# MJavaadAkhtar/GCN-max-cut

Hardware: AMD Instinct MI355X
Metric: training epochs/sec (n=1000 d=7 graphs) (higher is better)
Workload: dtype f32; 1 GPU; 160 x n=1000 d=7 regular graphs per GPU (BASELINE configs[3] on one GPU; 160 graphs per step), GCN 1000->500->3, batched steps, Adam lr 1e-3; graphs_per_gpu=160, rows_per_gpu=160000, nnz_per_gpu=1120000, hidden_dim=500, mode=batched, epoch_graphs=160, parallelism=single

## Files before the change

gcn-max-cut_amd/csrc/api.hip:

```cpp
#include "launchers.h"
#include <stdlib.h>

namespace {

int g_fuse = -1;
bool fuse_enabled() {
    if (g_fuse < 0) {
        g_fuse = 1;
#ifdef GMC_TUNING
        const char *e = getenv("GMC_FUSE");
        if (e && e[0] == '0') g_fuse = 0;
#endif
    }
    return g_fuse != 0;
}

struct Plan {
    int fs;
    bool fused;
    bool head_in_bwd;
    int zparts;
    int slices;
    int chunks;
};

Plan plan(const gmc_batch *b, int F, float dropout_p, bool fuse, bool train_step, bool dense = false,
          bool hard_loss = true) {
    Plan p{};
    p.zparts = 1;
    if (dense) return p;
    const bool dropout = dropout_p > 0.f;
    const GmcLdsGeom g = gmc_lds_geometry(b, F);
    bool lds = g.fits && !(g.ovf && (!fuse || dropout));
#ifdef GMC_TUNING
    static const bool forced_rows = [] {
        const char *e = getenv("GMC_SPMM_ALGO");
        return e && e[0] == 'r';
    }();
    if (forced_rows) lds = false;
#endif
    if (!lds) return p;
    p.fs = g.fs;
    p.slices = g.slices;
    p.chunks = gmc_dw1_chunks(b->B, true, g.slices);
    p.fused = fuse && !dropout;
    if (!dropout) p.zparts = gmc_lds_groups(b, F);
    p.head_in_bwd = train_step && hard_loss && p.fused && p.chunks == 1 && gmc_bwd1_takes_head(b);
    return p;
}

struct Workspace {
    Plan plan;
    long ld;
    float *T0;
    float *H;
    float *Z0;
    float *GY2;
    float *part;
    float *db2part;
    float *dw1part;
    float *W2s;
    size_t bytes;
};

bool dropout_on(const gmc_model *m) { return m->dropout_p > 0.f; }
int loss_kind_of(const gmc_model *m) { return (m->flags & GMC_MODEL_LOSS_EXPECTED) ? GMC_LOSS_EXPECTED_CUT : GMC_LOSS_CUT; }
unsigned long long dropout_seed(const gmc_model *m) { return ((unsigned long long)m->dropout_seed_hi << 32) | m->dropout_seed_lo; }

size_t align_up(size_t x) { return (x + 255) & ~(size_t)255; }

Workspace carve(const gmc_batch *b, const gmc_model *m, int training, void *base, bool train_step = false,
                bool dense = false) {
    Workspace w{};
    size_t off = 0;
    auto take = [&](size_t floats) {
        float *p = base ? reinterpret_cast<float *>(static_cast<char *>(base) + off) : nullptr;
        off += align_up(floats * sizeof(float));
        return p;
    };
// ... 18 lines not shown
    return w;
}

int check(const gmc_batch *b, const gmc_model *m, bool dense = false) {
    if (!b || !m) return GMC_ERR_NULL;
    if (b->abi != GMC_VERSION || m->abi != GMC_VERSION) return GMC_ERR_ABI;
    if (!b->goff || !b->rowptr || !b->gcol || !b->lcol || !b->dinv) return GMC_ERR_NULL;
    if (!m->W1 || !m->b1 || !m->W2 || !m->b2) return GMC_ERR_NULL;
    if (m->K != 3) return GMC_ERR_CLASSES;
    if (b->B < 0 || b->R < 0 || b->nnz < 0 || m->N <= 0 || m->F <= 0) return GMC_ERR_SHAPE;
    if (m->F % 4 || m->F > GMC_MAX_HIDDEN) return GMC_ERR_UNSUPPORTED;
    if (!(m->dropout_p >= 0.f && m->dropout_p < 1.f)) return GMC_ERR_SHAPE;
    if (m->W1_slab && !gmc_aligned16(m->W1_slab)) return GMC_ERR_ALIGN;
    if (b->B > 0 && (b->n_max < 3 || b->n_max > GMC_MAX_GRAPH_NODES)) return GMC_ERR_GRAPH_SIZE;
    if (!dense && b->n_max > m->N) return GMC_ERR_SHAPE;
    return GMC_OK;
}

int group_rows(const gmc_batch *b) { return b->uniform_n > 0 ? b->uniform_n : b->n_max; }


int aggregate(const gmc_batch *b, const Workspace &w, const float *X, float *Y, int F, const float *bias, int relu,
              const float *W2, float *Z0, int tag, hipStream_t st) {
    if (w.plan.fs)
        return gmc_spmm_lds_launch(b, X, w.ld, 1, 0, 0, b->dinv, bias, relu, Y, w.ld, 1, F, W2, Z0, tag, st);
    return gmc_spmm_launch(b->rowptr, b->gcol, nullptr, b->dinv, X, w.ld, bias, relu, Y, w.ld, b->R, F,
                           group_rows(b), W2, Z0, tag, st);
}

int forward_body(const gmc_batch *b, const gmc_model *m, const Workspace &w, hipStream_t st, const float *X = nullptr,
                 long ldx = 0) {
    const int F = m->F;
    if (w.plan.fused)
        return gmc_fwd1_lds_launch(b, m->W1, m->b1, m->W2, w.H, w.Z0, F, st, m->W1_slab, m->N);
    const int fs = w.plan.fs;
    int rc = X ? gmc_gemm_launch(0, 0, b->R, F, m->N, X, ldx, m->W1, F, b->dinv, w.T0, w.ld, st)
             : fs ? gmc_spmm_lds_launch(b, m->W1, F, 0, 1, 1, b->dinv, nullptr, 0, w.T0, w.ld, 1, F, nullptr,
                                        nullptr, GMC_K_GATHER_W1, st)
                  : gmc_spmm_launch(b->rowptr, b->lcol, b->vals, b->dinv, m->W1, F, nullptr, 0, w.T0, w.ld,
                                    b->R, F, group_rows(b), nullptr, nullptr, GMC_K_GATHER_W1, st);
    if (rc) return rc;
    if (dropout_on(m)) {
        rc = aggregate(b, w, w.T0, w.H, F, m->b1, 1, nullptr, nullptr, GMC_K_AGG_FWD, st);
        if (rc) return rc;
        rc = gmc_dropout_launch(w.H, b->R, F, fs, w.ld, m->dropout_p, dropout_seed(m), st);
        if (rc) return rc;
        return gmc_hw2_rows_launch(w.H, b->dinv, m->W2, w.Z0, b->R, F, fs, w.ld, st);
    }
    return aggregate(b, w, w.T0, w.H, F, m->b1, 1, m->W2, w.Z0, GMC_K_AGG_FWD, st);
}

struct AdamFuse {
    float *param = nullptr, *m = nullptr, *v = nullptr;
    double lr = 0, beta1 = 0, beta2 = 0, eps = 0;
    int *step_counter = nullptr;
    float *w1_slab = nullptr;
};

int backward_body(const gmc_batch *b, const gmc_model *m, const Workspace &w, float *grad,
                  hipStream_t st, const AdamFuse *af = nullptr, const float *loss_tail = nullptr,
                  const gmc_bwd1_head *head = nullptr, const float *X = nullptr, long ldx = 0, float *dX = nullptr,
                  long lddx = 0) {
    const long F = m->F;
    float *dW1 = grad, *db1 = grad + (long)m->N * F, *dW2 = db1 + F, *db2 = dW2 + F * 3;
    float *Gs = w.T0, *U = w.H;
    const float *W2b = m->W2;
    if (dropout_on(m)) {
// ... 79 lines not shown
}

extern "C" int gmc_probe_end(int32_t *tags, float *ms, int32_t max) {
    g_probe.on = false;
    const int n = (int)g_probe.used;
    if (n > 0) {
        hipError_t e = hipEventSynchronize(g_probe.pool[n - 1].b);
        if (e != hipSuccess) return -(int)e - 1000;
    }
    for (int i = 0; i < n && i < max; ++i) {
        float t = 0.f;
        (void)hipEventElapsedTime(&t, g_probe.pool[i].a, g_probe.pool[i].b);
        if (tags) tags[i] = g_probe.pool[i].tag;
        if (ms) ms[i] = t;
    }
    return n;
}

extern "C" int gmc_probe_flavours(int32_t *words, int32_t max) {
    if (g_probe.on) return GMC_ERR_UNSUPPORTED;
    const int n = (int)g_probe.used;
    for (int i = 0; i < n && i < max; ++i)
        if (words) words[i] = g_probe.pool[i].flv;
    return n;
}

extern "C" int gmc_lds_flavours(const gmc_batch *batch, int32_t F, int32_t one_graph_step, int32_t *words, int32_t max) {
    if (!batch) return GMC_ERR_NULL;
    if (batch->abi != GMC_VERSION) return GMC_ERR_ABI;
    if (F <= 0 || F % 4 || F > GMC_MAX_HIDDEN || max < 0 || batch->B < 0) return GMC_ERR_SHAPE;
    int out[6], n = 0;
    const Plan fused = plan(batch, F, 0.f, true, one_graph_step != 0), unfused = plan(batch, F, 0.f, false, false);
    if (fused.fused) {
        out[n++] = gmc_fwd1_flavour(batch, F);
        out[n++] = gmc_bwd1_flavour(batch, F, fused.head_in_bwd);
    }
    if (unfused.fs) {
        out[n++] = gmc_spmm_lds_flavour(batch, F, 1, 1, false);
        out[n++] = gmc_spmm_lds_flavour(batch, F, 0, 0, true);
        out[n++] = gmc_spmm_lds_flavour(batch, F, 0, 0, false);
        out[n++] = gmc_dw1_lds_flavour(batch, F);
    }
    for (int i = 0; i < n && i < max; ++i)
        if (words) words[i] = out[i];
    return n;
}

extern "C" int gmc_set_fuse(int on) {
    const int prev = fuse_enabled() ? 1 : 0;
    g_fuse = on ? 1 : 0;
    return prev;
}

extern "C" int gmc_version(void) { return GMC_VERSION; }

extern "C" const char *gmc_error_string(int code) {
    switch (code) {
        case GMC_OK: return "ok";
        case GMC_ERR_NULL: return "required pointer is NULL";
        case GMC_ERR_SHAPE: return "negative or inconsistent sizes";
        case GMC_ERR_CLASSES: return "number_classes must be 3 (override_fixed_nodes is 3-wide)";
        case GMC_ERR_ALIGN: return "pointer or leading dimension not 16-byte aligned";
        case GMC_ERR_WORKSPACE: return "workspace too small";
        case GMC_ERR_GRAPH_SIZE: return "graph has fewer than 3 or more than GMC_MAX_GRAPH_NODES nodes";
        case GMC_ERR_UNSUPPORTED: return "unsupported shape (the hidden width F must be a multiple of 4 and <= 4096 = GMC_MAX_HIDDEN)";
        case GMC_ERR_LOSS: return "unknown loss kind (GMC_LOSS_CUT = 0, GMC_LOSS_EXPECTED_CUT = 1)";
        case GMC_ERR_ABI: return "gmc_batch.abi / gmc_model.abi differs from the library's GMC_VERSION: rebuild the caller against this include/gcnmaxcut.h";
// ... 172 lines not shown
```

gcn-max-cut_amd/csrc/fwd1_lds.hip:

```cpp
#include "lds_tile.h"

#ifdef GMC_STAMP
extern "C" int gmc_debug_read_stamps_fwd(unsigned long long *out, int n) {
    return (int)hipMemcpyFromSymbol(out, HIP_SYMBOL(g_stamps), sizeof(unsigned long long) * n);
}
#endif

namespace {

template <int FS, int W, int ACC, bool HAS_VAL, int NS, bool OVF>
__global__ GMC_LDS_BOUNDS void fwd1_lds_kernel(TileArgs a) {
    STAMP_DECL;
    MARK(0);
    extern __shared__ __attribute__((aligned(16))) float lds[];
    constexpr int Q = FS / 4;
    constexpr int kRowsPerPass = kThreads / Q;
    constexpr int NT = (ACC * kRowsPerPass * (W / 8) + kThreads - 1) / kThreads;
    const int total = a.b.B * a.groups;
    const int it0 = (int)blockIdx.x * a.items_per_wg, it1 = min(total, it0 + a.items_per_wg);
    if (it0 >= it1) return;
    const int per = (a.slices + a.groups - 1) / a.groups;

    const int TF = (int)tile_floats(a.b.n_max, FS);
    float *bufA = lds, *bufB = lds + TF;
    unsigned short *nb = reinterpret_cast<unsigned short *>(lds + 2 * TF);
    constexpr bool CSL = W == 16;
    float4 *cst = reinterpret_cast<float4 *>(nb + (size_t)a.b.n_max * W);
    const int q = threadIdx.x % Q, lrow = threadIdx.x / Q;
    constexpr bool ovf = OVF;
    auto col_consts = [&](int cc) {
        float4 c = gmc::f4_zero();
        if (cc < a.F) {
            if (a.W2) { c.x = a.W2[(long)cc * 3]; c.y = a.W2[(long)cc * 3 + 1]; c.z = a.W2[(long)cc * 3 + 2]; }
            if (a.bias) c.w = a.bias[cc];
        }
        return c;
    };

    constexpr int kSlicesPerWin = kThreads / FS;
    auto load_window = [&](int win) {
        const int cc = win * kThreads + (int)threadIdx.x;
// ... 61 lines not shown
            for (int k = 0; k < NT; ++k) {
                const int i = tid + k * kThreads;
                pt[k] = i < n * (W / 8) ? src[i] : make_uint4(0, 0, 0, 0);
            }
            if constexpr (ovf) {
                ovf_blocks(a.b, tid, ol, orq);
                ovf_commit(a.b, n, tid, ol, orq);
                const int ob = orq.ob;
#pragma unroll
                for (int k = 0; k < ACC; ++k) {
                    const unsigned dsc = hp1[k] > hp0[k] ? (unsigned)(((hp1[k] - hp0[k]) << 12) | (hp0[k] - ob)) : 0u;
                    hub[k / 2] |= dsc << (16 * (k & 1));
                }
            }
#pragma unroll
            for (int k = 0; k < NT; ++k) {
                const int i = tid + k * kThreads;
                if (i < n * (W / 8)) reinterpret_cast<uint4 *>(nb)[i] = pt[k];
            }
        }
        if (tid < kPadRows * FS) {
            bufA[(long)n * FS + tid] = 0.f;
            bufB[(long)n * FS + tid] = 0.f;
        }
        gmc::v2f z01[ACC];
        float z2[ACC];
#pragma unroll
        for (int k = 0; k < ACC; ++k) { z01[k] = gmc::splat2(0.f); z2[k] = 0.f; }
        auto flush = [&](int grp) {
            if (a.Zpart) {
                float *zp = a.Zpart + ((long)grp * a.b.R + r0) * 3;
#pragma unroll
                for (int k = 0; k < ACC; ++k) {
                    float z0 = z01[k].x, z1 = z01[k].y, zz = z2[k];
                    z0 = gmc::xor_tree<Q / 2, 1>(z0); z1 = gmc::xor_tree<Q / 2, 1>(z1); zz = gmc::xor_tree<Q / 2, 1>(zz);
                    int l = lrow + k * kRowsPerPass;
                    asm volatile("" : "+v"(l));
                    if (q == 0 && l < n) {
                        zp[3 * l] = z0 * sc[k]; zp[3 * l + 1] = z1 * sc[k]; zp[3 * l + 2] = zz * sc[k];
                    }
                }
            }
#pragma unroll
            for (int k = 0; k < ACC; ++k) { z01[k] = gmc::splat2(0.f); z2[k] = 0.f; }
        };
        dma_wait();
        if (CSL && threadIdx.x < FS) cst[(s_lo & 1) * FS + threadIdx.x] = cn;
        STAMP(11);
        for (int s = s_lo; s < s_hi; ++s) {
            STAMP(0);
            if (s > s_lo && !ABL(1) && !ABL(2)) {
                vm_wait<ACC>();
                if (CSL && threadIdx.x < FS) cst[(s & 1) * FS + threadIdx.x] = cn;
            }
            STAMP(1);
            loop_barrier();
            STAMP(2);
            if (!CSL && s / kSlicesPerWin != win) {
                win = s / kSlicesPerWin;
                load_window(win);
            }
            if constexpr (W == 8) {
                uint4 ids = reinterpret_cast<const uint4 *>(nb)[min(lrow, n - 1)];
#pragma unroll
                for (int k = 0; k < ACC; ++k) {
                    const int l = lrow + k * kRowsPerPass;
                    const uint4 cur = ids;
                    if (k + 1 < ACC) ids = reinterpret_cast<const uint4 *>(nb)[min(l + kRowsPerPass, n - 1)];
                    const int lc = min(l, n - 1);
                    float4 t = ABL(5) ? make_float4(sc[k], sc[k], sc[k], sc[k])
                                      : gather_ids8<FS, HAS_VAL, NS>(bufA, cur, HAS_VAL ? wbase + (long)lc * W : nullptr, q);
                    t.x *= sc[k]; t.y *= sc[k]; t.z *= sc[k]; t.w *= sc[k];
// ... 13 lines not shown
            bool hub_any = false;
            if constexpr (ovf) {
                unsigned any = 0;
#pragma unroll
                for (int i = 0; i < (ACC + 1) / 2; ++i) any |= hub[i];
                hub_any = __builtin_amdgcn_ballot_w64(any != 0) != 0;
            }
            if (hub_any) {
                unsigned dk[ACC];
#pragma unroll
                for (int k = 0; k < ACC; ++k) dk[k] = lrow + k * kRowsPerPass < n ? desc_of(k) : 0u;
#pragma unroll
                for (int k = 0; k < ACC; ++k) {
                    const int lm = lrow + k * kRowsPerPass;
                    float4 mine = gmc::f4_zero();
                    for_hub_rows<FS, 0>(dk[k], lm, q, bufA, nullptr, ol, n, [&](int l, const float4 t) { if (lm == l) mine = t; });
                    if (dk[k] != 0) {
                        float4 *cell = reinterpret_cast<float4 *>(bufB) + lm * Q + q;
                        const float4 c = *cell;
                        *cell = make_float4(fmaf(mine.x, sc[k], c.x), fmaf(mine.y, sc[k], c.y), fmaf(mine.z, sc[k], c.z), fmaf(mine.w, sc[k], c.w));
                    }
                }
            }
            STAMP(3);
            loop_barrier();
            STAMP(4);
            if (s > s_lo && s % per == 0) flush(s / per - 1);
            if (s + 1 < s_hi && !ABL(1)) {
                dma(s + 1);
                if (CSL && threadIdx.x < FS) cn = col_consts((s + 1) * FS + (int)threadIdx.x);
            }
            STAMP(5);
            const int cb = (CSL ? (s & 1) : s - win * kSlicesPerWin) * FS + 4 * q;
            const float4 c0 = cst[cb], c1 = cst[cb + 1], c2 = cst[cb + 2], c3 = cst[cb + 3];
            const gmc::v2f w01[4] = {{c0.x, c0.y}, {c1.x, c1.y}, {c2.x, c2.y}, {c3.x, c3.y}};
            const float w2c[4] = {c0.z, c1.z, c2.z, c3.z};
            const gmc::v2f blo = {c0.w, c1.w}, bhi = {c2.w, c3.w};
            const bool col_pad = s * FS + 4 * q >= a.F;
            float *ydst = a.Y + (long)s * a.y_ss + 4 * q;
            float scm[ACC];
#pragma unroll
            for (int k = 0; k < ACC; ++k) scm[k] = col_pad ? 0.f : sc[k];
            auto emit = [&](int k, const gmc::v4f acc) {
                int l = min(lrow + k * kRowsPerPass, n - 1);
                if constexpr (ovf) asm volatile("" : "+v"(l));
                const gmc::v2f s2 = gmc::splat2(scm[k]);
                const gmc::v2f ylo = gmc::pk_fma((gmc::v2f){acc.x, acc.y}, s2, blo);
                const gmc::v2f yhi = gmc::pk_fma((gmc::v2f){acc.z, acc.w}, s2, bhi);
                float4 y;
                y.x = gmc::relu1(ylo.x); y.y = gmc::relu1(ylo.y); y.z = gmc::relu1(yhi.x); y.w = gmc::relu1(yhi.y);
                if (!ABL(2)) store_nt(ydst + (long)(r0 + l) * a.y_rs, y);
                if (ABL(3)) { z2[k] += y.x + y.y + y.z + y.w; return; }
                z01[k] = gmc::pk_fma(gmc::splat2(y.x), w01[0], z01[k]); z2[k] = fmaf(y.x, w2c[0], z2[k]);
                z01[k] = gmc::pk_fma(gmc::splat2(y.y), w01[1], z01[k]); z2[k] = fmaf(y.y, w2c[1], z2[k]);
                z01[k] = gmc::pk_fma(gmc::splat2(y.z), w01[2], z01[k]); z2[k] = fmaf(y.z, w2c[2], z2[k]);
                z01[k] = gmc::pk_fma(gmc::splat2(y.w), w01[3], z01[k]); z2[k] = fmaf(y.w, w2c[3], z2[k]);
            };
            uint4 ids2 = reinterpret_cast<const uint4 *>(nb)[min(lrow, n - 1)];
#pragma unroll
            for (int k = 0; k < ACC; ++k) {
                const int l = min(lrow + k * kRowsPerPass, n - 1);
                bool later = false;
                if constexpr (ovf) later = desc_of(k) != 0;
                if constexpr (W == 8) {
                    const uint4 cur = ids2;
                    if (k + 1 < ACC) ids2 = reinterpret_cast<const uint4 *>(nb)[min(l + kRowsPerPass, n - 1)];
                    const gmc::v4f h = ABL(4) ? (gmc::v4f)(__uint_as_float(cur.x)) : gather_ids8_pk<FS, NS>(bufB, cur, q);
                    if (!later) emit(k, h);
                } else {
                    const gmc::v4f h = gmc::f4v(gather_row<FS, W, false, NS>(bufB, nb, nullptr, l, q));
                    if (!later) emit(k, h);
                }
            }
            if (hub_any) {
#pragma unroll
                for (int k = 0; k < ACC; ++k) {
                    const int lm = min(lrow + k * kRowsPerPass, n - 1);
                    gmc::v4f h = (gmc::v4f)(0.f);
                    for_hub_rows<FS, W>(desc_of(k), lm, q, bufB, nb, ol, n, [&](int l, const float4 t) { if (lm == l) h = gmc::f4v(t); });
                    if (desc_of(k) != 0) emit(k, h);
                }
            }
            STAMP(6);
        }
        flush((s_hi - 1) / per);
        it = it_end;
    }
    STAMP(7);
    STAMP_FLUSH;
    MARK(3);
}

struct Fwd1Built {
    template <typename L> static constexpr bool has(L) {
        if (L::HEAD || L::EPI || L::SHARED || (L::HAS_VAL && L::OVF)) return false;
        return L::HAS_VAL || L::OVF ? L::NS == L::W : true;
    }
};

}

int gmc_fwd1_flavour(const gmc_batch *b, int F) {
    const GmcLdsGeom g = gmc_lds_geometry(b, F);
    if (!g.fits || F <= 0) return 0;
    if (g.W == 8 && (size_t)16 * kThreads > lds_consts(b->n_max, g.fs, 8)) return 0;
    if (g.slices * g.fs > GMC_MAX_HIDDEN) return 0;
    return flavour_word(GMC_FLV_FWD1, g.fs, g.W, g.acc, g.hv, g.ns, g.ovf) | flavour_per(gmc_lds_slices_per_group(b, F));
}

int gmc_fwd1_lds_launch(const gmc_batch *b, const float *W1, const float *b1, const float *W2, float *H,
                        float *Zpart, int F, hipStream_t st, const float *W1_slab, int N) {
    const int flv = gmc_fwd1_flavour(b, F);
    if (!flv) return GMC_ERR_UNSUPPORTED;
    if (b->B == 0) return GMC_OK;
    const int fs = GMC_FLV_FS(flv);
    const int slices = (F + fs - 1) / fs, groups = gmc_lds_groups(b, F);
    const int total = b->B * groups, cus = device_cus();
    const int ipw = (total + cus - 1) / cus, grid = (total + ipw - 1) / ipw;
    TileArgs a{*b, W1, (long)F, (long)fs, 1, b->ell_vals != nullptr, b->dinv, b1, 1, H, (long)fs, (long)b->R * fs,
               F, slices, groups, W2, Zpart, ipw, 0, 0, 0, 0};
    if (W1_slab) { a.X = W1_slab; a.x_rs = 16; a.x_slab16 = 1; a.x_rows = N; }
    size_t lds = lds_bytes(b->n_max, b->ell_width, fs);
    if (GMC_FLV_OVF(flv)) {
        const size_t own = ovf_own_bytes(0, b->n_max, b->ell_width, fs);
        if (own + ovf_desc_bytes(b->n_max) > kOvfLdsBytes) return GMC_ERR_UNSUPPORTED;
        a.own_lds = (int)own;
        a.ovf_cap = ovf_cap_blocks(own, b->n_max);
        lds = kOvfLdsBytes;
    }
    GmcProbeScope probe(GMC_K_FWD1_FUSED, st);
    return decode_flavour<Fwd1Built>(flv, [&](auto L) {
        using K = decltype(L);
        return launch_flv(flv, K::word(GMC_FLV_FWD1), fwd1_lds_kernel<K::FS, K::W, K::ACC, K::HAS_VAL, K::NS, K::OVF>,
                          grid, lds, st, a);
    });
}
```

gcn-max-cut_amd/csrc/launchers.h:

```cpp
#pragma once
#include "gmc_common.h"

struct GmcLdsGeom {
    bool fits;
    int fs;
    int W;
    int acc;
    int ns;
    bool hv;
    bool ovf;
    int slices;
};
GmcLdsGeom gmc_lds_geometry(const gmc_batch *b, int F);
bool gmc_lds_fits(const gmc_batch *b);
int gmc_lds_slices_per_group(const gmc_batch *b, int F);
int gmc_lds_groups(const gmc_batch *b, int F);
int device_cus(bool allow_override = true);

int gmc_fwd1_flavour(const gmc_batch *b, int F);
int gmc_bwd1_flavour(const gmc_batch *b, int F, bool head);
int gmc_spmm_lds_flavour(const gmc_batch *b, int F, int shared_src, int use_vals, bool epi);
int gmc_dw1_lds_flavour(const gmc_batch *b, int F);
bool gmc_bwd1_takes_head(const gmc_batch *b);

int gmc_fwd1_lds_launch(const gmc_batch *b, const float *W1, const float *b1, const float *W2, float *H, float *Zpart,
                        int F, hipStream_t st, const float *W1_slab, int N);
struct gmc_bwd1_head {
    const float *Z0; int zparts; const float *b2; float C; float *P; int *S; float *loss; float *db2part; int *tick;
};
int gmc_bwd1_lds_launch(const gmc_batch *b, const float *H, const float *GY2, const float *W2, float *dw1part,
                        float *colpart, int F, int chunks, int graphs_per_chunk, hipStream_t st,
                        const gmc_bwd1_head *head);
int gmc_finish_launch(const float *dw1part, const float *colpart, const float *db2part, int chunks, int n_max, int N,
                      int F, int B, float *grad, float *param, float *m, float *v, double lr, double beta1,
                      double beta2, double eps, int *step_counter, const float *loss_for_tail, hipStream_t st,
                      float *w1_slab);
int gmc_loss_tail_launch(const float *loss, int B, float *slot, hipStream_t st);

int gmc_spmm_launch(const int32_t *rowptr, const int32_t *col, const float *vals, const float *scale, const float *X,
                    int64_t ldx, const float *bias, int relu, float *Y, int64_t ldy, int32_t n_rows, int32_t F,
                    int32_t group_rows, const float *W2, float *Z0, int tag, hipStream_t st);
int gmc_spmm_lds_launch(const gmc_batch *b, const float *X, long ldx, int x_slab, int shared_src, int use_vals,
                        const float *scale, const float *bias, int relu, float *Y, long ldy, int y_slab, int F,
                        const float *W2, float *Zpart, int tag, hipStream_t st);

int gmc_dw1_chunks(int B, bool lds, int slices);
size_t gmc_dw1_scratch_floats(const gmc_batch *b, int N, int F, bool lds);
int gmc_dw1_launch(const gmc_batch *b, const float *U, long ldu, float *dW1, float *scratch, int N, int F, bool lds,
                   hipStream_t st);
int gmc_dw1_lds_launch(const gmc_batch *b, const float *U, long ldu, int u_slab, float *out, int F, int chunks,
                       int graphs_per_chunk, hipStream_t st);

inline bool gmc_loss_kind_ok(int kind) { return kind == GMC_LOSS_CUT || kind == GMC_LOSS_EXPECTED_CUT; }
int gmc_head_launch(const gmc_batch *batch, const float *Z0, int32_t z_parts, const float *b2, float C, float *P,
                    int32_t *S, float *loss, float *GY2, float *db2part, int *tick, hipStream_t st, int loss_kind);
int gmc_head_bwd_launch(const gmc_batch *batch, const float *P, const float *GP, float *GY2, float *db2part,
                        hipStream_t st);
int gmc_hidden_tiles(int R);
int gmc_hidden_slab_tiles(int R);
// ... 14 lines not shown
```

gcn-max-cut_amd/csrc/lds_tile.h:

```cpp
#pragma once
#include "gmc_common.h"
#include "launchers.h"
#include <stdlib.h>
#include <type_traits>


#ifdef GMC_STAMP
static __device__ unsigned long long g_stamps[4096 * 16];
#ifdef GMC_MARKS_ONLY
#define STAMP_DECL
#define STAMP(i)
#define STAMP_FLUSH
#else
#define STAMP_DECL unsigned long long st_last = __builtin_amdgcn_s_memtime(); unsigned long long st_acc[12] = {}
#define STAMP(i)                                                     \
    do {                                                             \
        __builtin_amdgcn_sched_barrier(0);                           \
        const unsigned long long st_now = __builtin_amdgcn_s_memtime(); \
        st_acc[i] += st_now - st_last;                               \
        st_last = st_now;                                            \
        __builtin_amdgcn_sched_barrier(0);                           \
    } while (0)
#define STAMP_FLUSH                                                                    \
    do {                                                                               \
// ... 21 lines not shown

namespace {

#ifndef GMC_LDS_THREADS
#define GMC_LDS_THREADS 1024
#endif
constexpr int kThreads = GMC_LDS_THREADS;
#ifndef GMC_LDS_WAVES_PER_EU
#define GMC_LDS_WAVES_PER_EU 4
#endif
#define GMC_LDS_BOUNDS __launch_bounds__(kThreads) __attribute__((amdgpu_waves_per_eu(GMC_LDS_WAVES_PER_EU, GMC_LDS_WAVES_PER_EU)))

struct TileArgs {
    gmc_batch b;
    const float *X;
    long x_rs, x_ss;
    int shared_src;
    int use_vals;
    const float *scale;
    const float *bias;
    int relu;
    float *Y;
    long y_rs, y_ss;
    int F;
    int slices;
    int groups;
    const float *W2;
    float *Zpart;
    int items_per_wg;
    int x_slab16;
    int x_rows;
    int ovf_cap;
    int own_lds;
};

__device__ __forceinline__ int sload(const int32_t *p, int index) {
    int v;
    asm volatile("s_load_dword %0, %1, 0x0\n\ts_waitcnt lgkmcnt(0)" : "=s"(v) : "s"(p + index) : "memory");
    return v;
}

__device__ __forceinline__ void tile_of(int b, int B, int S, int &g, int &s) {
    const int full = (B / 8) * 8 * S;
    if (b < full) {
        const int xcd = b & 7, j = b >> 3;
        g = (j / S) * 8 + xcd;
        s = j % S;
    } else {
        const int t = b - full;
        const int rem = B - (B / 8) * 8;
        g = (B / 8) * 8 + t % rem;
        s = t / rem;
    }
}


constexpr int kPadRows = 4;
__host__ __device__ inline size_t tile_floats(int n_max, int FS) { return (size_t)(n_max + kPadRows) * FS; }
constexpr int kMaxSlicesPerWg = 8;
__host__ __device__ inline size_t lds_consts(int n_max, int FS, int W) {
    if (W == 16) return (size_t)16 * kMaxSlicesPerWg * FS;
    const size_t cols = (size_t)16 * 1024, rows = (size_t)16 * (n_max + kPadRows);
    return cols > rows ? cols : rows;
}
size_t lds_bytes(int n_max, int W, int FS) {
    return 2 * tile_floats(n_max, FS) * 4 + (size_t)n_max * W * 2 + lds_consts(n_max, FS, W);
// ... 415 lines not shown
```

gcn-max-cut_amd/hip.py:

```python
from __future__ import annotations

import ctypes as C
import os
from typing import Optional

import torch

_PKG = os.path.dirname(os.path.abspath(__file__))
LIB_PATH = os.environ.get("GCN_MAXCUT_LIB") or os.path.join(_PKG, "lib", "libgcnmaxcut_hip.so")

SYMBOLS = (
    "gmc_version", "gmc_error_string", "gmc_spmm_f32", "gmc_dense_hw2_f32", "gmc_head_f32",
    "gmc_adam_f32", "gmc_workspace_bytes", "gmc_forward", "gmc_train_fwd_bwd",
    "gmc_backward_from_gp", "gmc_probe_begin", "gmc_probe_end", "gmc_set_fuse", "gmc_decode_sample_f32", "gmc_adam_devstep_f32", "gmc_ell_arrange_host", "gmc_ell_slots_for", "gmc_train_step_f32",
    "gmc_adam_devstep_model_f32", "gmc_w1_slab_floats", "gmc_w1_slab_f32", "gmc_host_device_pointer", "gmc_publish_f32",
    "gmc_publish_adam_devstep_model_f32", "gmc_probe_flavours", "gmc_lds_flavours", "gmc_refine_order_host",
    "gmc_refine_local_f32", "gmc_refine_anneal_f32", "gmc_refine_anneal_staged",
    "gmc_gemm_f32", "gmc_workspace_bytes_features", "gmc_forward_features", "gmc_backward_features_from_gp",
    "gmc_head_loss_f32", "gmc_train_step_loss_f32", "gmc_cut_loss_f32",
)

MAX_GRAPH_NODES = 4096
ANNEAL_LEVELS = 1024
MODEL_GRAD_TAIL = 1
# ... 147 lines not shown
    raise RuntimeError(f"{what}: HIP error {rc}: {msg}")


def ptr(t: Optional[torch.Tensor]) -> Optional[int]:
    if t is None:
        return None
    if not t.is_cuda:
        raise HipExtensionError("tensor is not on a HIP device")
    if not t.is_contiguous():
        raise ValueError("tensor must be contiguous")
    return t.data_ptr()


def mapped_ptr(t: torch.Tensor) -> Optional[int]:
    lib = load()
    if not (t.device.type == "cpu" and t.is_pinned() and t.is_contiguous()):
        return None
    out = C.c_void_p()
    if lib.gmc_host_device_pointer(C.c_void_p(t.data_ptr()), C.byref(out)) != 0 or not out.value:
        return None
    return int(out.value)


def stream() -> int:
    return torch.cuda.current_stream().cuda_stream


KERNEL_TAGS = ("gather_w1", "agg_fwd", "head", "hidden_bwd", "colsum", "agg_bwd", "dw1", "dw1_fold",
               "adam", "spmm_user", "dense_mfma", "bwd1_fused", "fwd1_fused", "decode", "finish",
               "refine", "anneal")
PROBE_TAGS = KERNEL_TAGS + ("gemm",)


FLAVOUR_KERNELS = {1: "fwd1_lds", 2: "bwd1_lds", 3: "bwd1_reg", 4: "spmm_lds", 5: "dw1_lds"}


def flavour_fields(word: int) -> dict:
    return dict(kernel=FLAVOUR_KERNELS.get(word & 7, "?"), FS=word >> 3 & 0x7f, W=word >> 10 & 0x1f,
                ACC=word >> 15 & 0xf, NS=word >> 19 & 0x1f, HAS_VAL=word >> 24 & 1, OVF=word >> 25 & 1,
                HEAD=word >> 26 & 1, EPI=word >> 27 & 1, SHARED=word >> 28 & 1, PER=1 << (word >> 29 & 3))


def lds_flavours(batch_struct: GmcBatch, F: int, one_graph_step: bool = False) -> list:
    words = (C.c_int32 * 8)()
    n = load().gmc_lds_flavours(C.byref(batch_struct), int(F), int(bool(one_graph_step)), words, 8)
    if n < 0:
        check(n, "gmc_lds_flavours")
    return [int(words[i]) for i in range(n)]


class Probe:

    def __init__(self, capacity: int):
        self.capacity, self.records, self.flavours = capacity, [], []

    def __enter__(self):
        check(load().gmc_probe_begin(self.capacity), "gmc_probe_begin")
        return self

    def __exit__(self, *exc):
        tags = (C.c_int32 * self.capacity)()
        ms = (C.c_float * self.capacity)()
        n = load().gmc_probe_end(tags, ms, self.capacity)
        if n < 0:
            raise RuntimeError(f"gmc_probe_end failed ({n})")
        self.records = [(PROBE_TAGS[tags[i]], float(ms[i])) for i in range(min(n, self.capacity))]
        words = (C.c_int32 * self.capacity)()
# ... 6 lines not shown
```

include/gcnmaxcut.h:

```cpp
#ifndef GCNMAXCUT_H
#define GCNMAXCUT_H

#include <stddef.h>
#include <stdint.h>

#ifdef __cplusplus
extern "C" {
#endif

#define GMC_VERSION 200

typedef void *gmc_stream_t;

enum {
    GMC_OK = 0,
    GMC_ERR_NULL = -1,
    GMC_ERR_SHAPE = -2,
    GMC_ERR_CLASSES = -3,
    GMC_ERR_ALIGN = -4,
    GMC_ERR_WORKSPACE = -5,
    GMC_ERR_GRAPH_SIZE = -6,
    GMC_ERR_UNSUPPORTED = -7,
    GMC_ERR_ABI = -8,
    GMC_ERR_LOSS = -9
// ... 62 lines not shown
    GMC_K_BWD1_FUSED = 11,
    GMC_K_FWD1_FUSED = 12,
    GMC_K_DECODE = 13,
    GMC_K_FINISH = 14,
    GMC_K_REFINE = 15,
    GMC_K_ANNEAL = 16,
    GMC_K_GEMM = 17,
    GMC_K_COUNT = 18
};

int gmc_set_fuse(int on);

int gmc_probe_begin(int32_t capacity);
int gmc_probe_end(int32_t *tags, float *ms, int32_t max);
int gmc_probe_flavours(int32_t *words, int32_t max);

#define GMC_FLV_KERNEL(w) ((w) & 0x7)
#define GMC_FLV_FS(w) (((w) >> 3) & 0x7f)
#define GMC_FLV_W(w) (((w) >> 10) & 0x1f)
#define GMC_FLV_ACC(w) (((w) >> 15) & 0xf)
#define GMC_FLV_NS(w) (((w) >> 19) & 0x1f)
#define GMC_FLV_HAS_VAL(w) (((w) >> 24) & 1)
#define GMC_FLV_OVF(w) (((w) >> 25) & 1)
#define GMC_FLV_HEAD(w) (((w) >> 26) & 1)
#define GMC_FLV_EPI(w) (((w) >> 27) & 1)
#define GMC_FLV_SHARED(w) (((w) >> 28) & 1)
#define GMC_FLV_PER(w) (1 << (((w) >> 29) & 3))
#define GMC_FLV_PER_MASK (3 << 29)
enum {
    GMC_FLV_FWD1 = 1,
    GMC_FLV_BWD1 = 2,
    GMC_FLV_BWD1_REG = 3,
    GMC_FLV_SPMM = 4,
    GMC_FLV_DW1 = 5
};
int gmc_lds_flavours(const gmc_batch *batch, int32_t F, int32_t one_graph_step, int32_t *words, int32_t max);


int gmc_spmm_f32(const int32_t *rowptr, const int32_t *col, const float *vals,
                 const float *scale, const float *X, int64_t ldx, const float *bias, int relu,
                 float *Y, int64_t ldy, int32_t n_rows, int32_t F, int32_t group_rows,
                 const float *W2, float *Z0, gmc_stream_t stream);

int gmc_dense_hw2_f32(const float *H, int64_t ldh, const float *dinv, const float *W2,
                      float *Z0, int32_t n_rows, int32_t F, gmc_stream_t stream);

int gmc_gemm_f32(int32_t ta, int32_t tb, int32_t M, int32_t Nc, int32_t K, const float *A, int64_t lda,
                 const float *B, int64_t ldb, const float *scale, float *C, int64_t ldc, gmc_stream_t stream);

int gmc_head_f32(const gmc_batch *batch, const float *Z0, int32_t z_parts, const float *b2, float C,
                 float *P, int32_t *S, float *loss, float *GY2, float *db2part, gmc_stream_t stream);

int gmc_head_loss_f32(const gmc_batch *batch, const float *Z0, int32_t z_parts, const float *b2, float C,
                      int32_t loss_kind, float *P, int32_t *S, float *loss, float *GY2, float *db2part,
                      gmc_stream_t stream);

int gmc_cut_loss_f32(const gmc_batch *batch, const float *P, float C, int32_t loss_kind, float *loss, float *GP,
                     gmc_stream_t stream);

int gmc_adam_f32(float *param, const float *grad, float *m, float *v, int64_t count, double lr,
                 double beta1, double beta2, double eps, int32_t step, gmc_stream_t stream);

int gmc_adam_devstep_f32(float *param, const float *grad, float *m, float *v, int64_t count, double lr,
                         double beta1, double beta2, double eps, int32_t *step_counter,
                         gmc_stream_t stream);

int gmc_adam_devstep_model_f32(float *param, const float *grad, float *m, float *v, int32_t N, int32_t F,
// ... 76 lines not shown
```

Baseline: 3846 epochs/s (1 epoch = 160 graphs).

## Add slice-major fused forward kernel that keeps one feature slice resident across graphs

Adds a new fused layer-1 forward kernel in which each workgroup owns one feature slice and a chunk of graphs. It loads the W1 slice into LDS once and reuses it across consecutive graphs, prefetching the next graph's ELL rows and scales. The planner selects it when the geometry matches (W=8, ACC=4, no overflow) and occupancy heuristics hold, with Z partials written per slice. The aim is to avoid reloading W1 per graph and to improve load balance, at the cost of more Z partial groups for the head to reduce.

Result: slower. 3502 epochs/s (1 epoch = 160 graphs) (-9.0%).

```diff
diff --git a/gcn-max-cut_amd/csrc/api.hip b/gcn-max-cut_amd/csrc/api.hip
--- a/gcn-max-cut_amd/csrc/api.hip
+++ b/gcn-max-cut_amd/csrc/api.hip
@@ -20,6 +20,7 @@
     bool fused;
     bool head_in_bwd;
     int zparts;
+    int fwd_chunks;
     int slices;
     int chunks;
 };
@@ -45,6 +46,15 @@
     p.chunks = gmc_dw1_chunks(b->B, true, g.slices);
     p.fused = fuse && !dropout;
     if (!dropout) p.zparts = gmc_lds_groups(b, F);
+    if (p.fused && gmc_fwd1_slice_flavour(b, F)) {
+        const int fc = gmc_fwd1_slice_chunks(b->B, g.slices), cus = device_cus(false);
+        const long items = (long)b->B * p.zparts;
+        const bool small = (long)b->B * g.slices < cus / 2;
+        if (b->B >= 2 * fc && (small || (long)g.slices * fc >= (items < cus ? items : cus))) {
+            p.fwd_chunks = fc;
+            p.zparts = g.slices;
+        }
+    }
     p.head_in_bwd = train_step && hard_loss && p.fused && p.chunks == 1 && gmc_bwd1_takes_head(b);
     return p;
 }
@@ -129,7 +139,7 @@
                  long ldx = 0) {
     const int F = m->F;
     if (w.plan.fused)
-        return gmc_fwd1_lds_launch(b, m->W1, m->b1, m->W2, w.H, w.Z0, F, st, m->W1_slab, m->N);
+        return gmc_fwd1_lds_launch(b, m->W1, m->b1, m->W2, w.H, w.Z0, F, st, m->W1_slab, m->N, w.plan.fwd_chunks);
     const int fs = w.plan.fs;
     int rc = X ? gmc_gemm_launch(0, 0, b->R, F, m->N, X, ldx, m->W1, F, b->dinv, w.T0, w.ld, st)
              : fs ? gmc_spmm_lds_launch(b, m->W1, F, 0, 1, 1, b->dinv, nullptr, 0, w.T0, w.ld, 1, F, nullptr,
@@ -275,7 +285,7 @@
     int out[6], n = 0;
     const Plan fused = plan(batch, F, 0.f, true, one_graph_step != 0), unfused = plan(batch, F, 0.f, false, false);
     if (fused.fused) {
-        out[n++] = gmc_fwd1_flavour(batch, F);
+        out[n++] = fused.fwd_chunks ? gmc_fwd1_slice_flavour(batch, F) : gmc_fwd1_flavour(batch, F);
         out[n++] = gmc_bwd1_flavour(batch, F, fused.head_in_bwd);
     }
     if (unfused.fs) {
diff --git a/gcn-max-cut_amd/csrc/fwd1_lds.hip b/gcn-max-cut_amd/csrc/fwd1_lds.hip
--- a/gcn-max-cut_amd/csrc/fwd1_lds.hip
+++ b/gcn-max-cut_amd/csrc/fwd1_lds.hip
@@ -7,6 +7,35 @@
 #endif
 
 namespace {
+
+struct ColConsts {
+    gmc::v2f w01[4];
+    float w2c[4];
+    gmc::v2f blo, bhi;
+};
+__device__ __forceinline__ ColConsts col_consts_of(const float4 c0, const float4 c1, const float4 c2, const float4 c3) {
+    return ColConsts{{{c0.x, c0.y}, {c1.x, c1.y}, {c2.x, c2.y}, {c3.x, c3.y}}, {c0.z, c1.z, c2.z, c3.z}, {c0.w, c1.w}, {c2.w, c3.w}};
+}
+__device__ __forceinline__ float4 h_row(const ColConsts &c, const gmc::v4f acc, float scm) {
+    const gmc::v2f s2 = gmc::splat2(scm);
+    const gmc::v2f ylo = gmc::pk_fma((gmc::v2f){acc.x, acc.y}, s2, c.blo);
+    const gmc::v2f yhi = gmc::pk_fma((gmc::v2f){acc.z, acc.w}, s2, c.bhi);
+    float4 y;
+    y.x = gmc::relu1(ylo.x); y.y = gmc::relu1(ylo.y); y.z = gmc::relu1(yhi.x); y.w = gmc::relu1(yhi.y);
+    return y;
+}
+__device__ __forceinline__ void z_row(const ColConsts &c, const float4 y, gmc::v2f &z01, float &z2) {
+    z01 = gmc::pk_fma(gmc::splat2(y.x), c.w01[0], z01); z2 = fmaf(y.x, c.w2c[0], z2);
+    z01 = gmc::pk_fma(gmc::splat2(y.y), c.w01[1], z01); z2 = fmaf(y.y, c.w2c[1], z2);
+    z01 = gmc::pk_fma(gmc::splat2(y.z), c.w01[2], z01); z2 = fmaf(y.z, c.w2c[2], z2);
+    z01 = gmc::pk_fma(gmc::splat2(y.w), c.w01[3], z01); z2 = fmaf(y.w, c.w2c[3], z2);
+}
+template <int Q>
+__device__ __forceinline__ void z_fold(const gmc::v2f z01, const float z2, const float sc, float (&z)[3]) {
+    z[0] = gmc::xor_tree<Q / 2, 1>(z01.x) * sc;
+    z[1] = gmc::xor_tree<Q / 2, 1>(z01.y) * sc;
+    z[2] = gmc::xor_tree<Q / 2, 1>(z2) * sc;
+}
 
 template <int FS, int W, int ACC, bool HAS_VAL, int NS, bool OVF>
 __global__ GMC_LDS_BOUNDS void fwd1_lds_kernel(TileArgs a) {
@@ -134,12 +163,12 @@
                 float *zp = a.Zpart + ((long)grp * a.b.R + r0) * 3;
 #pragma unroll
                 for (int k = 0; k < ACC; ++k) {
-                    float z0 = z01[k].x, z1 = z01[k].y, zz = z2[k];
-                    z0 = gmc::xor_tree<Q / 2, 1>(z0); z1 = gmc::xor_tree<Q / 2, 1>(z1); zz = gmc::xor_tree<Q / 2, 1>(zz);
+                    float z[3];
+                    z_fold<Q>(z01[k], z2[k], sc[k], z);
                     int l = lrow + k * kRowsPerPass;
                     asm volatile("" : "+v"(l));
                     if (q == 0 && l < n) {
-                        zp[3 * l] = z0 * sc[k]; zp[3 * l + 1] = z1 * sc[k]; zp[3 * l + 2] = zz * sc[k];
+                        zp[3 * l] = z[0]; zp[3 * l + 1] = z[1]; zp[3 * l + 2] = z[2];
                     }
                 }
             }
@@ -219,10 +248,7 @@
             }
             STAMP(5);
             const int cb = (CSL ? (s & 1) : s - win * kSlicesPerWin) * FS + 4 * q;
-            const float4 c0 = cst[cb], c1 = cst[cb + 1], c2 = cst[cb + 2], c3 = cst[cb + 3];
-            const gmc::v2f w01[4] = {{c0.x, c0.y}, {c1.x, c1.y}, {c2.x, c2.y}, {c3.x, c3.y}};
-            const float w2c[4] = {c0.z, c1.z, c2.z, c3.z};
-            const gmc::v2f blo = {c0.w, c1.w}, bhi = {c2.w, c3.w};
+            const ColConsts cw = col_consts_of(cst[cb], cst[cb + 1], cst[cb + 2], cst[cb + 3]);
             const bool col_pad = s * FS + 4 * q >= a.F;
             float *ydst = a.Y + (long)s * a.y_ss + 4 * q;
             float scm[ACC];
@@ -231,17 +257,10 @@
             auto emit = [&](int k, const gmc::v4f acc) {
                 int l = min(lrow + k * kRowsPerPass, n - 1);
                 if constexpr (ovf) asm volatile("" : "+v"(l));
-                const gmc::v2f s2 = gmc::splat2(scm[k]);
-                const gmc::v2f ylo = gmc::pk_fma((gmc::v2f){acc.x, acc.y}, s2, blo);
-                const gmc::v2f yhi = gmc::pk_fma((gmc::v2f){acc.z, acc.w}, s2, bhi);
-                float4 y;
-                y.x = gmc::relu1(ylo.x); y.y = gmc::relu1(ylo.y); y.z = gmc::relu1(yhi.x); y.w = gmc::relu1(yhi.y);
+                const float4 y = h_row(cw, acc, scm[k]);
                 if (!ABL(2)) store_nt(ydst + (long)(r0 + l) * a.y_rs, y);
                 if (ABL(3)) { z2[k] += y.x + y.y + y.z + y.w; return; }
-                z01[k] = gmc::pk_fma(gmc::splat2(y.x), w01[0], z01[k]); z2[k] = fmaf(y.x, w2c[0], z2[k]);
-                z01[k] = gmc::pk_fma(gmc::splat2(y.y), w01[1], z01[k]); z2[k] = fmaf(y.y, w2c[1], z2[k]);
-                z01[k] = gmc::pk_fma(gmc::splat2(y.z), w01[2], z01[k]); z2[k] = fmaf(y.z, w2c[2], z2[k]);
-                z01[k] = gmc::pk_fma(gmc::splat2(y.w), w01[3], z01[k]); z2[k] = fmaf(y.w, w2c[3], z2[k]);
+                z_row(cw, y, z01[k], z2[k]);
             };
             uint4 ids2 = reinterpret_cast<const uint4 *>(nb)[min(lrow, n - 1)];
 #pragma unroll
@@ -278,10 +297,125 @@
     MARK(3);
 }
 
+template <int FS, int ACC, int NS>
+__global__ GMC_LDS_BOUNDS void fwd1_slice_kernel(TileArgs a) {
+    extern __shared__ __attribute__((aligned(16))) float lds[];
+    constexpr int W = 8;
+    constexpr int Q = FS / 4;
+    constexpr int kRowsPerPass = kThreads / Q;
+    int chunk, s;
+    tile_of((int)blockIdx.x, a.chunks, a.slices, chunk, s);
+    const int g0 = chunk * a.items_per_wg, g1 = min(a.b.B, g0 + a.items_per_wg);
+    if (g0 >= g1) return;
+    const int n_max = a.b.n_max;
+    const int TF = (int)tile_floats(n_max, FS);
+    float *bufA = lds, *bufB = lds + TF;
+    const int q = threadIdx.x % Q, lrow = threadIdx.x / Q;
+    const int f0 = s * FS + 4 * q;
+    int r0 = a.b.goff[g0], n = a.b.goff[g0 + 1] - r0;
+    int nn = g0 + 1 < g1 ? a.b.goff[g0 + 2] - (r0 + n) : 0;
+    {
+        const int cs = min(f0, ((a.F + 15) & ~15) - 4);
+        const long off = a.x_slab16 ? gmc::slab16_index(0, cs, a.x_rows) : (long)min(f0, a.F - 4);
+        dma_tile<FS, ACC>(a.X + off, a.x_rs, n_max, true, lrow, bufA);
+    }
+    uint4 idr[ACC], idn[ACC];
+    float sc[ACC], scn[ACC];
+    auto request_rows = [&](int r0, int n) {
+#pragma unroll
+        for (int k = 0; k < ACC; ++k)
+            idn[k] = *reinterpret_cast<const uint4 *>(a.b.ell + (long)(r0 + min(lrow + k * kRowsPerPass, n - 1)) * W);
+#pragma unroll
+        for (int k = 0; k < ACC; ++k) scn[k] = a.scale[r0 + min(lrow + k * kRowsPerPass, n - 1)];
+    };
+    request_rows(r0, n);
+    float4 cc[4];
+#pragma unroll
+    for (int j = 0; j < 4; ++j) {
+        const int c = min(f0 + j, a.F - 1);
+        cc[j] = make_float4(a.W2[(long)c * 3], a.W2[(long)c * 3 + 1], a.W2[(long)c * 3 + 2], a.bias[c]);
+    }
+#pragma unroll
+    for (int j = 0; j < 4; ++j)
+        if (f0 + j >= a.F) cc[j] = gmc::f4_zero();
+    const ColConsts cw = col_consts_of(cc[0], cc[1], cc[2], cc[3]);
+    if (threadIdx.x < kPadRows * FS) {
+        bufA[(long)n_max * FS + threadIdx.x] = 0.f;
+        bufB[(long)n_max * FS + threadIdx.x] = 0.f;
+    }
+    const bool col_pad = f0 >= a.F;
+    float *ydst = a.Y + (long)s * a.y_ss + 4 * q;
+    float *zdst = a.Zpart + (long)s * a.b.R * 3;
+    float zo[ACC][3];
+    int rz = 0, nz = 0;
+    auto store_z = [&]() {
+#pragma unroll
+        for (int k = 0; k < ACC; ++k) {
+            const int l = lrow + k * kRowsPerPass;
+            if (q == 0 && l < nz) {
+                float *zp = zdst + (long)(rz + l) * 3;
+                zp[0] = zo[k][0]; zp[1] = zo[k][1]; zp[2] = zo[k][2];
+            }
+        }
+    };
+    dma_wait();
+    for (int g = g0; g < g1; ++g) {
+#pragma unroll
+        for (int k = 0; k < ACC; ++k)
+            asm volatile("" : "+v"(idn[k].x), "+v"(idn[k].y), "+v"(idn[k].z), "+v"(idn[k].w), "+v"(scn[k]));
+        if (g > g0) store_z();
+#pragma unroll
+        for (int k = 0; k < ACC; ++k) { idr[k] = idn[k]; sc[k] = scn[k]; }
+        if (n < n_max) {
+            const unsigned un = (unsigned)n, up = (unsigned)(n_max - n);
+            auto move = [&](unsigned pk) {
+                unsigned lo = pk & 0xffffu, hi = pk >> 16;
+                lo += lo >= un ? up : 0u;
+                hi += hi >= un ? up : 0u;
+                return lo | hi << 16;
+            };
+#pragma unroll
+            for (int k = 0; k < ACC; ++k) idr[k] = make_uint4(move(idr[k].x), move(idr[k].y), move(idr[k].z), move(idr[k].w));
+        }
+        loop_barrier();
+#pragma unroll
+        for (int k = 0; k < ACC; ++k) {
+            const int lc = min(lrow + k * kRowsPerPass, n - 1);
+            float4 t = ABL(5) ? make_float4(sc[k], sc[k], sc[k], sc[k]) : gather_ids8<FS, false, NS>(bufA, idr[k], nullptr, q);
+            t.x *= sc[k]; t.y *= sc[k]; t.z *= sc[k]; t.w *= sc[k];
+            reinterpret_cast<float4 *>(bufB)[lc * Q + q] = t;
+        }
+        loop_barrier();
+        request_rows(nn > 0 ? r0 + n : r0, nn > 0 ? nn : n);
+        gmc::v2f z01[ACC];
+        float z2[ACC];
+#pragma unroll
+        for (int k = 0; k < ACC; ++k) {
+            const int l = min(lrow + k * kRowsPerPass, n - 1);
+            const gmc::v4f h = ABL(4) ? (gmc::v4f)(__uint_as_float(idr[k].x)) : gather_ids8_pk<FS, NS>(bufB, idr[k], q);
+            const float4 y = h_row(cw, h, col_pad ? 0.f : sc[k]);
+            if (!ABL(2)) store_nt(ydst + (long)(r0 + l) * a.y_rs, y);
+            z01[k] = gmc::splat2(0.f); z2[k] = 0.f;
+            z_row(cw, y, z01[k], z2[k]);
+        }
+#pragma unroll
+        for (int k = 0; k < ACC; ++k) z_fold<Q>(z01[k], z2[k], sc[k], zo[k]);
+        rz = r0; nz = n;
+        const int n2 = g + 2 < g1 ? sload(a.b.goff, g + 3) - (r0 + n + nn) : 0;
+        r0 += n; n = nn; nn = n2;
+    }
+    store_z();
+}
+
 struct Fwd1Built {
     template <typename L> static constexpr bool has(L) {
         if (L::HEAD || L::EPI || L::SHARED || (L::HAS_VAL && L::OVF)) return false;
         return L::HAS_VAL || L::OVF ? L::NS == L::W : true;
+    }
+};
+struct Fwd1SliceBuilt {
+    template <typename L> static constexpr bool has(L) {
+        return L::W == 8 && L::ACC == 4 && !L::HAS_VAL && !L::OVF && !L::HEAD && !L::EPI && !L::SHARED;
     }
 };
 
@@ -295,8 +429,38 @@
     return flavour_word(GMC_FLV_FWD1, g.fs, g.W, g.acc, g.hv, g.ns, g.ovf) | flavour_per(gmc_lds_slices_per_group(b, F));
 }
 
+int gmc_fwd1_slice_flavour(const gmc_batch *b, int F) {
+    const GmcLdsGeom g = gmc_lds_geometry(b, F);
+    if (!g.fits || F <= 0 || F > 1024 || g.W != 8 || g.hv || g.ovf || g.acc != 4) return 0;
+    return flavour_word(GMC_FLV_FWD1_SLICE, g.fs, g.W, g.acc, false, g.ns, false);
+}
+
+int gmc_fwd1_slice_chunks(int B, int slices) {
+    int c = gmc_dw1_chunks(B, true, slices);
+    if (c > 8) c = 8;
+    const int per = (B + c - 1) / c;
+    return per > 0 ? (B + per - 1) / per : 1;
+}
+
 int gmc_fwd1_lds_launch(const gmc_batch *b, const float *W1, const float *b1, const float *W2, float *H,
-                        float *Zpart, int F, hipStream_t st, const float *W1_slab, int N) {
+                        float *Zpart, int F, hipStream_t st, const float *W1_slab, int N, int slice_chunks) {
+    if (slice_chunks > 0) {
+        const int flv = gmc_fwd1_slice_flavour(b, F);
+        if (!flv || slice_chunks > b->B || !b1 || !W2 || !Zpart) return GMC_ERR_UNSUPPORTED;
+        const int fs = GMC_FLV_FS(flv), slices = (F + fs - 1) / fs;
+        const int per = (b->B + slice_chunks - 1) / slice_chunks;
+        if ((b->B + per - 1) / per != slice_chunks) return GMC_ERR_UNSUPPORTED;
+        TileArgs a{*b, W1, (long)F, (long)fs, 1, 0, b->dinv, b1, 1, H, (long)fs, (long)b->R * fs,
+                   F, slices, slices, W2, Zpart, per, 0, 0, 0, 0, slice_chunks};
+        if (W1_slab) { a.X = W1_slab; a.x_rs = 16; a.x_slab16 = 1; a.x_rows = N; }
+        const size_t lds = 2 * tile_floats(b->n_max, fs) * 4;
+        GmcProbeScope probe(GMC_K_FWD1_FUSED, st);
+        return decode_flavour<Fwd1SliceBuilt>(flv, [&](auto L) {
+            using K = decltype(L);
+            return launch_flv(flv, K::word(GMC_FLV_FWD1_SLICE), fwd1_slice_kernel<K::FS, K::ACC, K::NS>,
+                              slices * slice_chunks, lds, st, a);
+        });
+    }
     const int flv = gmc_fwd1_flavour(b, F);
     if (!flv) return GMC_ERR_UNSUPPORTED;
     if (b->B == 0) return GMC_OK;
@@ -305,7 +469,7 @@
     const int total = b->B * groups, cus = device_cus();
     const int ipw = (total + cus - 1) / cus, grid = (total + ipw - 1) / ipw;
     TileArgs a{*b, W1, (long)F, (long)fs, 1, b->ell_vals != nullptr, b->dinv, b1, 1, H, (long)fs, (long)b->R * fs,
-               F, slices, groups, W2, Zpart, ipw, 0, 0, 0, 0};
+               F, slices, groups, W2, Zpart, ipw, 0, 0, 0, 0, 0};
     if (W1_slab) { a.X = W1_slab; a.x_rs = 16; a.x_slab16 = 1; a.x_rows = N; }
     size_t lds = lds_bytes(b->n_max, b->ell_width, fs);
     if (GMC_FLV_OVF(flv)) {
diff --git a/gcn-max-cut_amd/csrc/launchers.h b/gcn-max-cut_amd/csrc/launchers.h
--- a/gcn-max-cut_amd/csrc/launchers.h
+++ b/gcn-max-cut_amd/csrc/launchers.h
@@ -18,13 +18,15 @@
 int device_cus(bool allow_override = true);
 
 int gmc_fwd1_flavour(const gmc_batch *b, int F);
+int gmc_fwd1_slice_flavour(const gmc_batch *b, int F);
 int gmc_bwd1_flavour(const gmc_batch *b, int F, bool head);
 int gmc_spmm_lds_flavour(const gmc_batch *b, int F, int shared_src, int use_vals, bool epi);
 int gmc_dw1_lds_flavour(const gmc_batch *b, int F);
 bool gmc_bwd1_takes_head(const gmc_batch *b);
 
 int gmc_fwd1_lds_launch(const gmc_batch *b, const float *W1, const float *b1, const float *W2, float *H, float *Zpart,
-                        int F, hipStream_t st, const float *W1_slab, int N);
+                        int F, hipStream_t st, const float *W1_slab, int N, int slice_chunks);
+int gmc_fwd1_slice_chunks(int B, int slices);
 struct gmc_bwd1_head {
     const float *Z0; int zparts; const float *b2; float C; float *P; int *S; float *loss; float *db2part; int *tick;
 };
diff --git a/gcn-max-cut_amd/csrc/lds_tile.h b/gcn-max-cut_amd/csrc/lds_tile.h
--- a/gcn-max-cut_amd/csrc/lds_tile.h
+++ b/gcn-max-cut_amd/csrc/lds_tile.h
@@ -77,6 +77,7 @@
     int x_rows;
     int ovf_cap;
     int own_lds;
+    int chunks;
 };
 
 __device__ __forceinline__ int sload(const int32_t *p, int index) {
diff --git a/gcn-max-cut_amd/hip.py b/gcn-max-cut_amd/hip.py
--- a/gcn-max-cut_amd/hip.py
+++ b/gcn-max-cut_amd/hip.py
@@ -203,7 +203,7 @@
 PROBE_TAGS = KERNEL_TAGS + ("gemm",)
 
 
-FLAVOUR_KERNELS = {1: "fwd1_lds", 2: "bwd1_lds", 3: "bwd1_reg", 4: "spmm_lds", 5: "dw1_lds"}
+FLAVOUR_KERNELS = {1: "fwd1_lds", 2: "bwd1_lds", 3: "bwd1_reg", 4: "spmm_lds", 5: "dw1_lds", 6: "fwd1_slice"}
 
 
 def flavour_fields(word: int) -> dict:
diff --git a/include/gcnmaxcut.h b/include/gcnmaxcut.h
--- a/include/gcnmaxcut.h
+++ b/include/gcnmaxcut.h
@@ -118,7 +118,8 @@
     GMC_FLV_BWD1 = 2,
     GMC_FLV_BWD1_REG = 3,
     GMC_FLV_SPMM = 4,
-    GMC_FLV_DW1 = 5
+    GMC_FLV_DW1 = 5,
+    GMC_FLV_FWD1_SLICE = 6
 };
 int gmc_lds_flavours(const gmc_batch *batch, int32_t F, int32_t one_graph_step, int32_t *words, int32_t max);
 
```
